# iucario/WorkoutDetector

Measured on AMD Instinct MI355X. Metric: clips/sec (8x3x224x224 TSM-R50), higher is better.
Workload: dtype f32

## Files before the change

### workoutdetector_amd/csrc/tsm_engine.hip

```cpp
#include <hip/hip_runtime.h>

#include <sys/stat.h>

#include <algorithm>
#include <cerrno>
#include <cmath>
#include <cstdio>
#include <cstdlib>
#include <cstring>
#include <map>
#include <string>
#include <vector>

#include "../../include/tsm_hip.h"
#include "tsm_host_util.h"
#include "tsm_kernels.h"

#ifndef TSM_BUILD_ID
#define TSM_BUILD_ID __DATE__ "/" __TIME__
#endif

namespace {

using namespace tsm_host;
// ... 97 lines not shown
  std::string err;
  hipStream_t stream = nullptr;
  bool finalized = false;
  int prec = tsm::kPrecF32;
  float *d_tap = nullptr;
  std::map<std::string, HostTensor> tensors;
  std::vector<ConvLayer> convs;
  std::vector<Block> blocks;
  float *d_fcw = nullptr, *d_fcb = nullptr;
  float *d_in = nullptr;
  float *d_in4 = nullptr;
  float *buf[5] = {nullptr, nullptr, nullptr, nullptr, nullptr};
  float *d_pooled = nullptr, *d_logits = nullptr;
  float *d_partial = nullptr;
  size_t partial_elems = 0;
  size_t buf_elems = 0;
  int h1 = 0, w1 = 0, hp = 0, wp = 0;
  hipEvent_t ev0 = nullptr, ev1 = nullptr;
  bool have_time = false;
  std::vector<void *> allocs;
  bool poison = false;
  std::vector<GuardBuf> guards;
  std::map<int, std::vector<int>> tile_cache;
  bool autotune = true;
  bool stem_pool = true;
  bool stem_direct = true;
  bool stem_planar = true;
  std::string tune_path, tune_sig;
  int force_tile = 0, force_code = -1;
  int fuse23 = -1;
  int fuse_block = -1;
  int fuse31 = -1;
  int fuse_front = -1;
  int walk = -1;
  int n_cu = 256;
  int timing_left = 0;
  bool timing_only3x3 = false;
  std::vector<std::vector<hipEvent_t>> timing;
  std::vector<hipEvent_t> event_pool;
  std::vector<hipEvent_t> *cur_timing = nullptr;
};

namespace {

int fail(tsm_engine *e, int code, const std::string &msg) {
  if (e) e->err = msg; else g_create_error = msg;
  return code;
}

#define TSM_HIP(e, call)                                                                        \
  do {                                                                                          \
    hipError_t _st = (call);                                                                    \
    if (_st != hipSuccess)                                                                      \
      return fail((e), TSM_ERR_HIP, std::string(#call) + ": " + hipGetErrorString(_st));        \
  } while (0)

void build_topology(tsm_engine *e) {
  e->convs.clear();
  e->blocks.clear();
  ConvLayer stem;
  stem.wkey = "base_model.conv1.weight";
  stem.bnp = "base_model.bn1";
  stem.cin = 3; stem.cout = 64; stem.k = 7; stem.stride = 2;
  stem.cp = 4;
  stem.kp = e->prec == tsm::kPrecF32 ? round_up(7 * 7 * 4, 32) : round_up(7 * 4 * 8, e->prec == tsm::kPrecBf16 ? 64 : 32);
  e->convs.push_back(stem);
// ... 342 lines not shown
            tsm::bneck_ws_valid(L.pb.cin, L.pb.N, L.pb.H, L.pb.W, L.pb.T, L.pb.fold) && !want(".conv1") && !want(".conv2");
  f.front = bf16 && blk.stride == 2 && c1.cin == 256 && c1.cout == 128 && c2.cin == 128 && c2.cout == 128 && e->fuse_front != 0 &&
            tsm::front_s2_valid(L.pfr.N, L.pfr.H, L.pfr.W, L.pfr.T, L.pfr.fold) && !want(".conv1");
  f.conv23 = (blk.d_w3f != nullptr || (bf16 && blk.cmid == 64 && tsm::conv23_ws_valid(nn, hh, ww))) && e->fuse23 != 0 &&
             !want(".conv2");
  f.conv31 = bf16 && blk.down < 0 && k + 1 < e->blocks.size() && e->blocks[k + 1].conv3 >= 0 && e->fuse31 != 0 &&
             tsm::conv31_valid(L.q);
  return f;
}

struct BlockPlan {
  bool block = false, front = false, conv1_done = false, conv23 = false, conv31_next = false;
};

std::vector<BlockPlan> plan_forward(const tsm_engine *e, const std::vector<int> *codes, int nn, const char *stage) {
  std::vector<BlockPlan> plan(e->blocks.size());
  int hh = e->hp, ww = e->wp;
  for (size_t k = 0; k < e->blocks.size(); ++k) {
    const Block &blk = e->blocks[k];
    const BlockForms can = fused_forms(e, k, nn, hh, ww, stage);
    auto chosen = [&](int force, int conv, int bit) { return force == 1 || (codes && ((*codes)[conv] & bit)); };
    BlockPlan &p = plan[k];
    p.conv1_done = k > 0 && plan[k - 1].conv31_next;
    if (can.block && chosen(e->fuse_block, blk.conv1, kCodeBlock)) p.block = true;
    else if (can.front && !p.conv1_done && chosen(e->fuse_front, blk.conv1, kCodeFront)) p.front = true;
    else if (can.conv23 && chosen(e->fuse23, blk.conv2, kCodeConv23)) p.conv23 = true;
    else if (can.conv31 && chosen(e->fuse31, blk.conv3, kCodeConv31)) p.conv31_next = true;
    hh = (hh + 2 - 3) / blk.stride + 1;
    ww = (ww + 2 - 3) / blk.stride + 1;
  }
  return plan;
}

struct Forward {
  tsm_engine *e;
  hipStream_t s;
  const char *stage;
  Tap *tap;
  int T, shiftT, prec;
  float *t1, *t2, *idb;
  std::vector<int> *tiles = nullptr;
  bool tuning = false;
  bool tapped = false;
  int flip = 0;
  int prev31 = -1;
  BlockLaunches prev;

  Forward(tsm_engine *e_, hipStream_t s_, const char *stage_, Tap *tap_)
      : e(e_), s(s_), stage(stage_), tap(tap_), T(e_->cfg.num_segments), shiftT(e_->cfg.is_shift ? T : 0), prec(e_->prec),
        t1(e_->buf[2]), t2(e_->buf[3]), idb(e_->buf[4]) {}

  int dir(int d) const { return e->walk >= 0 ? e->walk : d; }
  int next_dir() { return dir(flip ^= 1); }
  bool want(const std::string &name) const { return stage && name == stage; }
  int hit(const float *p, int64_t a, int64_t b, int64_t c, int64_t d) {
    tap->ptr = p; tap->shape[0] = a; tap->shape[1] = b; tap->shape[2] = c; tap->shape[3] = d; tap->hit = true;
    tapped = true;
    return TSM_OK;
  }
  hipError_t launch_code(tsm::ConvParams p, int ks, int code);
  hipError_t launch_pair(const tsm::ConvParams &a, int ks_a, int code_a, const tsm::ConvParams &b, int ks_b, int code_b) {
    const hipError_t st = launch_code(a, ks_a, code_a);
    return st != hipSuccess ? st : launch_code(b, ks_b, code_b);
  }
  template <class A, class B>
  int fused_wins(A &&many, B &&one, bool *wins) {
    float many_ms = 0.f, one_ms = 0.f;
    int rc = time_best_of(e, s, many, &many_ms);
    if (!rc) rc = time_best_of(e, s, one, &one_ms);
    *wins = one_ms < many_ms;
    return rc;
  }
  int conv(int idx, tsm::ConvParams p, int ks, bool is3x3);
  int run_basic(size_t k, int nn, float *x, float *y, int hh, int ww);
  int run_block(size_t k, const BlockPlan &plan, int nn, float *x, float *y, int hh, int ww);
  int tune_block(size_t k, int nn, float *x, float *y, int hh, int ww);
};

hipError_t Forward::launch_code(tsm::ConvParams p, int ks, int code) {
  return launch_conv_code(p, ks, code, e->d_partial, e->partial_elems, e->n_cu, s);
}

int Forward::conv(int idx, tsm::ConvParams p, int ks, bool is3x3) {
  p.reverse = next_dir();
  if (!tuning) {
    int code = tiles ? (*tiles)[idx] : 0;
    if (e->force_tile) code = e->force_tile;
    if (e->force_code >= 0) code = e->force_code;
    TSM_LAUNCH_K(e, s, is3x3, launch_code(p, ks, checked_code(p, code)));
    return TSM_OK;
  }
  std::vector<int> cands;
  if (p.kseg_len > 0) {
    const size_t need = (size_t)tsm::conv_num_segments(p) * p.M * p.Cout;
    const long tiles64 = (long)((p.M + 63) / 64) * (p.Cout / 64);
    for (int t : {(int)tsm::kTile64x64, (int)tsm::kTile32x32}) {
      cands.push_back(t);
      if (need <= e->partial_elems && tiles64 < 4L * e->n_cu) cands.push_back(t | kCodeSplitK);
    }
    int tail_from = 0;
    if (tail_split_from(p, e->n_cu, e->partial_elems, &tail_from)) cands.push_back((int)tsm::kTile64x64 | kCodeTailK);
  } else {
    for (int t = 1; t < tsm::kNumTiles; ++t)
      if (tsm::conv_tile_valid(p, t)) cands.push_back(t);
  }
  float best_ms = 0.f;
  int best = 0;
  for (int t : cands) {
    float ms = 0.f;
    const int rc = time_best_of(e, s, [&] { return launch_code(p, ks, t); }, &ms);
    if (rc) return rc;
    if (best == 0 || ms < best_ms) {
      best = t;
      best_ms = ms;
    }
  }
  (*tiles)[idx] = best;
  return TSM_OK;
}

int Forward::run_basic(size_t k, int nn, float *x, float *y, int hh, int ww) {
  const Block &blk = e->blocks[k];
  const std::string &name = blk.name;
  const ConvLayer &c1 = e->convs[blk.conv1], &c2 = e->convs[blk.conv2];
  const int ho = (hh + 2 - 3) / blk.stride + 1, wo = (ww + 2 - 3) / blk.stride + 1;
  const float *identity = x;
  if (blk.down >= 0) {
    tsm::ConvParams pd = make_params(e->convs[blk.down], x, nullptr, idb, nn, hh, ww, false, block_shift(e) ? shiftT : 0,
                                     e->cfg.shift_div, prec);
    int rcd = conv(blk.down, pd, 1, false);
    if (rcd) return rcd;
    identity = idb;
  }
  tsm::ConvParams p1 = make_params(c1, x, nullptr, t1, nn, hh, ww, true, shiftT, e->cfg.shift_div, prec);
  int rc1 = conv(blk.conv1, p1, 3, true);
  if (rc1) return rc1;
  if (want(name + ".conv1")) return hit(t1, nn, ho, wo, c1.cout);
// ... 6 lines not shown
  if (rc2) return rc2;
  if (want(name)) return hit(y, nn, ho, wo, c2.cout);
  return TSM_OK;
}

int Forward::run_block(size_t k, const BlockPlan &plan, int nn, float *x, float *y, int hh, int ww) {
  const Block &blk = e->blocks[k];
  const std::string &name = blk.name;
  const int c1out = e->convs[blk.conv1].cout, c2out = e->convs[blk.conv2].cout, c3out = e->convs[blk.conv3].cout;
  const int ho = (hh + 2 - 3) / blk.stride + 1, wo = (ww + 2 - 3) / blk.stride + 1;
  BlockLaunches L = block_launches(e, k, nn, x, y, t1, t2, hh, ww);
  if (blk.down >= 0) skip_slots(e, 1);
  if (plan.block) {
    L.pb.reverse = next_dir();
    TSM_LAUNCH(e, s, tsm::launch_bneck_ws(L.pb, s));
    skip_slots(e, 2);
    return want(name) ? hit(y, nn, ho, wo, c3out) : TSM_OK;
  }
  if (plan.front) {
    L.pfr.reverse = next_dir();
    TSM_LAUNCH(e, s, tsm::launch_front_s2(L.pfr, s));
    next_dir();
    skip_slots(e, 1);
  } else {
    if (plan.conv1_done) {
      skip_slots(e, 1);
    } else {
      int rc1 = conv(blk.conv1, L.p1, 1, false);
      if (rc1) return rc1;
    }
    if (want(name + ".conv1")) return hit(t1, nn, hh, ww, c1out);
    if (plan.conv23) {
      L.pf.reverse = next_dir();
      TSM_LAUNCH_K(e, s, true, tsm::launch_conv23_fused(L.pf, blk.cmid, blk.cout3, prec, s));
      skip_slots(e, 1);
      return want(name) ? hit(y, nn, ho, wo, c3out) : TSM_OK;
    }
    int rc2 = conv(blk.conv2, L.p2, 3, true);
    if (rc2) return rc2;
  }
  if (want(name + ".conv2")) return hit(t2, nn, ho, wo, c2out);
  if (plan.conv31_next) {
    L.q.reverse = next_dir();
    TSM_LAUNCH(e, s, tsm::launch_conv31_fused(L.q, s));
  } else {
    int rc3 = conv(blk.conv3, L.p3, 1, false);
    if (rc3) return rc3;
  }
  return want(name) ? hit(y, nn, ho, wo, c3out) : TSM_OK;
}

int Forward::tune_block(size_t k, int nn, float *x, float *y, int hh, int ww) {
  const Block &blk = e->blocks[k];
  std::vector<int> &codes = *tiles;
  const BlockForms can = fused_forms(e, k, nn, hh, ww, nullptr);
  BlockLaunches L = block_launches(e, k, nn, x, y, t1, t2, hh, ww);
  const int r1 = flip ^ 1;
  bool wins = false;
  int rc = conv(blk.conv1, L.p1, 1, false);
  if (rc) return rc;
  L.p1.reverse = dir(r1);
  if (prev31 >= 0 && e->fuse31 < 0) {
    const int conv3 = e->blocks[prev31].conv3, code3 = codes[conv3], code1 = codes[blk.conv1];
    tsm::ConvParams pc = L.p1;
    pc.reverse = dir(prev.p3.reverse ^ 1);
    prev.q.reverse = prev.p3.reverse;
    rc = fused_wins([&] { return launch_pair(prev.p3, 1, code3, pc, 1, code1); },
                    [&] { return tsm::launch_conv31_fused(prev.q, s); }, &wins);
    if (rc) return rc;
    if (wins) codes[conv3] |= kCodeConv31;
  }
  rc = conv(blk.conv2, L.p2, 3, true);
  if (rc) return rc;
  L.p2.reverse = dir(r1 ^ 1);
  if (can.front && e->fuse_front < 0) {
    const int code1 = codes[blk.conv1], code2 = codes[blk.conv2];
    L.pfr.reverse = dir(r1);
    rc = fused_wins([&] { return launch_pair(L.p1, 1, code1, L.p2, 3, code2); },
                    [&] { return tsm::launch_front_s2(L.pfr, s); }, &wins);
    if (rc) return rc;
    if (wins) codes[blk.conv1] |= kCodeFront;
  }
  rc = conv(blk.conv3, L.p3, 1, false);
  if (rc) return rc;
  L.p3.reverse = dir(r1);
  prev31 = can.conv31 ? (int)k : -1;
  prev = L;
  const int code1 = codes[blk.conv1], code2 = codes[blk.conv2], code3 = codes[blk.conv3];
  L.pf.reverse = dir(r1 ^ 1);
  L.pb.reverse = dir(r1);
  auto pair = [&] { return launch_pair(L.p2, 3, code2, L.p3, 1, code3); };
  auto fused23 = [&] { return tsm::launch_conv23_fused(L.pf, blk.cmid, blk.cout3, prec, s); };
  bool use_fused = can.conv23 && e->fuse23 == 1;
  if (can.conv23 && e->fuse23 < 0) {
    rc = fused_wins(pair, fused23, &use_fused);
    if (rc) return rc;
    if (use_fused) codes[blk.conv2] |= kCodeConv23;
  }
  if (can.block && e->fuse_block < 0) {
    rc = fused_wins([&] {
      const hipError_t st = launch_code(L.p1, 1, code1);
      return st != hipSuccess ? st : use_fused ? fused23() : pair();
    }, [&] { return tsm::launch_bneck_ws(L.pb, s); }, &wins);
    if (rc) return rc;
    if (wins) codes[blk.conv1] |= kCodeBlock;
  }
  return TSM_OK;
}

int run_forward(tsm_engine *e, const float *d_clips, int layout, int n_clips, float *d_logits,
                hipStream_t s, const char *stage, Tap *tap) {
  const tsm_config &cfg = e->cfg;
  const int T = cfg.num_segments, n = n_clips * T;
  Forward f(e, s, stage, tap);
  if (e->autotune && !stage) {
    auto it = e->tile_cache.find(tile_bucket(n_clips) * T);
    if (it == e->tile_cache.end()) {
      it = e->tile_cache.emplace(tile_bucket(n_clips) * T, std::vector<int>(e->convs.size(), 0)).first;
      f.tuning = true;
    }
    f.tiles = &it->second;
  }

  const int prec = e->prec;
  const float *in4 = e->d_in4;
  const bool pool_stem = e->stem_direct && e->stem_pool && !f.want("conv1");
  const bool planar = layout == TSM_LAYOUT_NTCHW && e->stem_planar && pool_stem && !f.want("input") &&
                      (double)cfg.height * cfg.width * 12.0 < 2.0e9 && (reinterpret_cast<uintptr_t>(d_clips) & 15u) == 0;
  if (layout >= TSM_LAYOUT_NTHWC4 || planar) {
    in4 = d_clips;
// ... 131 lines not shown
  if (cfg->height < 32 || cfg->width < 32)
    return fail(nullptr, TSM_ERR_INVALID_ARG, "height/width must be >= 32");
  {
    const int64_t rows = (int64_t)cfg->max_clips * cfg->num_segments * ((cfg->height + 1) / 2) * ((cfg->width + 1) / 2);
    if (rows >= (int64_t)1 << 31)
      return fail(nullptr, TSM_ERR_CAPACITY, "max_clips * num_segments * (H/2) * (W/2) must stay below 2^31");
  }
  if (cfg->shift_div <= 0 || (64 % cfg->shift_div) != 0 || (64 / cfg->shift_div) % 4 != 0)
    return fail(nullptr, TSM_ERR_UNSUPPORTED, "shift_div must divide 64 with fold % 4 == 0 (8 or 16... )");
  if (cfg->dtype != TSM_DTYPE_F32 && cfg->dtype != TSM_DTYPE_BF16X3 && cfg->dtype != TSM_DTYPE_BF16)
    return fail(nullptr, TSM_ERR_UNSUPPORTED, "dtype must be TSM_DTYPE_F32, TSM_DTYPE_BF16X3 or TSM_DTYPE_BF16");
  if (cfg->dtype != TSM_DTYPE_F32 && (64 / cfg->shift_div) % 8 != 0)
    return fail(nullptr, TSM_ERR_UNSUPPORTED, "the bf16 formats need fold % 8 == 0 (shift_div <= 8)");
  int ndev = 0;
  hipError_t st = hipGetDeviceCount(&ndev);
  if (st != hipSuccess || ndev <= 0)
    return fail(nullptr, TSM_ERR_HIP, std::string("no HIP device: ") + hipGetErrorString(st));
  if (cfg->device_id < 0 || cfg->device_id >= ndev) return fail(nullptr, TSM_ERR_INVALID_ARG, "bad device_id");
  tsm_engine *e = new tsm_engine();
  e->cfg = *cfg;
  e->prec = cfg->dtype == TSM_DTYPE_BF16X3 ? tsm::kPrecBf16x3
            : cfg->dtype == TSM_DTYPE_BF16 ? tsm::kPrecBf16 : tsm::kPrecF32;
  if (const char *at = getenv("TSM_AUTOTUNE")) e->autotune = atoi(at) != 0;
  if (const char *sd = getenv("TSM_STEM_DIRECT")) e->stem_direct = atoi(sd) != 0;
  if (const char *sp = getenv("TSM_STEM_POOL")) e->stem_pool = atoi(sp) != 0;
  if (const char *pl = getenv("TSM_STEM_PLANAR")) e->stem_planar = atoi(pl) != 0;
  if (const char *ft = getenv("TSM_CONV_TILE")) e->force_tile = tsm::conv_tile_from_name(ft);
  if (const char *fc = getenv("TSM_CONV_CODE")) e->force_code = atoi(fc);
  if (const char *f23 = getenv("TSM_FUSE_CONV23")) e->fuse23 = atoi(f23) != 0;
  if (const char *fb = getenv("TSM_FUSE_BLOCK")) e->fuse_block = atoi(fb) != 0;
  if (const char *f31 = getenv("TSM_FUSE_C3C1")) e->fuse31 = atoi(f31) != 0;
  if (const char *ff = getenv("TSM_FUSE_FRONT")) e->fuse_front = atoi(ff) != 0;
  if (const char *wk = getenv("TSM_WALK")) e->walk = atoi(wk) != 0;
  if (const char *po = getenv("TSM_POISON")) e->poison = atoi(po) != 0;
  {
    const char *tc = getenv("TSM_TUNE_CACHE");
    if (tc) {
      if (*tc && strcmp(tc, "0") != 0 && strcmp(tc, "off") != 0) e->tune_path = tc;
    } else {
      e->tune_path = default_tune_cache_path();
    }
  }
  build_topology(e);
  st = hipSetDevice(cfg->device_id);
  if (st == hipSuccess) st = hipStreamCreateWithFlags(&e->stream, hipStreamNonBlocking);
  if (st == hipSuccess) st = hipDeviceGetAttribute(&e->n_cu, hipDeviceAttributeMultiprocessorCount, cfg->device_id);
  if (st == hipSuccess) st = hipEventCreate(&e->ev0);
  if (st == hipSuccess) st = hipEventCreate(&e->ev1);
  if (st != hipSuccess) {
    g_create_error = std::string("engine init: ") + hipGetErrorString(st);
    delete e;
    return TSM_ERR_HIP;
  }
  if (!e->tune_path.empty()) {
    hipDeviceProp_t prop;
    e->tune_sig = "abi" + std::to_string(TSM_ABI_VERSION) + " build " TSM_BUILD_ID " " +
                  (hipGetDeviceProperties(&prop, cfg->device_id) == hipSuccess ? std::string(prop.gcnArchName) : "?") +
                  " cu" + std::to_string(e->n_cu) +
                  " T" + std::to_string(cfg->num_segments) + " " + std::to_string(cfg->height) + "x" +
                  std::to_string(cfg->width) + " dtype" + std::to_string(cfg->dtype) + " shift" +
                  std::to_string(cfg->is_shift ? cfg->shift_div : 0) + " fuse" + std::to_string(e->fuse23) + "/" + std::to_string(e->fuse_block) + "/" + std::to_string(e->fuse31) + "/" + std::to_string(e->fuse_front) +
                  " stem" + std::to_string(e->stem_direct ? 1 : 0) +
                  std::to_string(e->stem_pool ? 1 : 0) + std::to_string(e->stem_planar ? 1 : 0);
    e->tune_sig_base = e->tune_sig.size();
  }
  *out = e;
  return TSM_OK;
}

int tsm_set_backbone(tsm_engine *e, int32_t depth) {
  if (!e) return TSM_ERR_INVALID_ARG;
  if (e->weights_started || e->finalized)
    return fail(e, TSM_ERR_INVALID_ARG, "tsm_set_backbone must come before the first tsm_set_tensor");
  if (!find_backbone(depth)) return fail(e, TSM_ERR_UNSUPPORTED, "depth must be 18, 34 or 50");
  if (find_backbone(depth)->basic && e->width != 64)
    return fail(e, TSM_ERR_UNSUPPORTED, "a BasicBlock backbone (depth 18 / 34) has no bottleneck width: the engine's is " +
                                            std::to_string(e->width));
  e->depth = depth;
  build_topology(e);
  retag_tune_sig(e);
  return TSM_OK;
}

int tsm_set_bottleneck_width(tsm_engine *e, int32_t width_per_group) {
  if (!e) return TSM_ERR_INVALID_ARG;
  if (e->weights_started || e->finalized)
    return fail(e, TSM_ERR_INVALID_ARG, "tsm_set_bottleneck_width must come before the first tsm_set_tensor");
  if (width_per_group != 64 && width_per_group != 128)
    return fail(e, TSM_ERR_UNSUPPORTED, "width_per_group must be 64 or 128 (wide_resnet50_2)");
  if (width_per_group != 64 && find_backbone(e->depth)->basic)
    return fail(e, TSM_ERR_UNSUPPORTED, "width_per_group 128 needs a Bottleneck backbone (depth 50): torchvision's BasicBlock "
                                        "supports 64 only");
  e->width = width_per_group;
  build_topology(e);
  retag_tune_sig(e);
  return TSM_OK;
// ... 292 lines not shown
  e->timing_only3x3 = only_conv3x3 != 0;
  for (auto &v : e->timing)
    for (hipEvent_t ev : v)
      if (ev) e->event_pool.push_back(ev);
  e->timing.clear();
  e->timing.reserve(64);
  e->timing_left = n_forwards;
  return TSM_OK;
}

int tsm_layer_times(tsm_engine *e, int32_t forward_index, float *ms_out, int32_t cap, int32_t *n_out) {
  if (!e || !ms_out || !n_out) return TSM_ERR_INVALID_ARG;
  if (forward_index < 0 || forward_index >= (int32_t)e->timing.size())
    return fail(e, TSM_ERR_INVALID_ARG, "no timing recorded for that forward");
  const std::vector<hipEvent_t> &ev = e->timing[forward_index];
  const int n = (int)ev.size() / 2;
  *n_out = n;
  if (n > cap) return fail(e, TSM_ERR_CAPACITY, "ms_out too small");
  for (int i = 0; i < n; ++i) {
    ms_out[i] = -1.f;
    if (!ev[2 * i] || !ev[2 * i + 1]) continue;
    TSM_HIP(e, hipEventSynchronize(ev[2 * i + 1]));
    TSM_HIP(e, hipEventElapsedTime(&ms_out[i], ev[2 * i], ev[2 * i + 1]));
  }
  return TSM_OK;
}

int tsm_conv_tiles(tsm_engine *e, int32_t n_clips, int32_t *tiles_out, int32_t cap, int32_t *n_out) {
  if (!e || !tiles_out || !n_out) return TSM_ERR_INVALID_ARG;
  std::vector<int> codes(e->convs.size(), 0);
  auto it = e->tile_cache.find(tile_bucket(n_clips) * e->cfg.num_segments);
  if (it != e->tile_cache.end()) {
    const std::vector<BlockPlan> plan = plan_forward(e, &it->second, n_clips * e->cfg.num_segments, nullptr);
    for (size_t i = 0; i < codes.size(); ++i) codes[i] = it->second[i] & ~kCodeFused;
    for (size_t k = 0; k < e->blocks.size(); ++k) {
      const Block &b = e->blocks[k];
      const BlockPlan &p = plan[k];
      codes[b.conv1] |= it->second[b.conv1] & ((p.block ? kCodeBlock : 0) | (p.front ? kCodeFront : 0));
      if (p.conv23) codes[b.conv2] |= it->second[b.conv2] & kCodeConv23;
      if (p.conv31_next) codes[b.conv3] |= it->second[b.conv3] & kCodeConv31;
    }
  }
  std::vector<int> order{0};
  for (const Block &b : e->blocks)
    for (int ci : {b.down, b.conv1, b.conv2, b.conv3})
      if (ci >= 0) order.push_back(ci);
  *n_out = (int32_t)order.size();
  if ((int)order.size() > cap) return fail(e, TSM_ERR_CAPACITY, "tiles_out too small");
  for (size_t i = 0; i < order.size(); ++i) tiles_out[i] = codes[order[i]];
  return TSM_OK;
}

float tsm_last_forward_ms(tsm_engine *e) {
  if (!e || !e->have_time) return -1.f;
  if (hipEventSynchronize(e->ev1) != hipSuccess) return -1.f;
  float ms = -1.f;
  if (hipEventElapsedTime(&ms, e->ev0, e->ev1) != hipSuccess) return -1.f;
  return ms;
}


int tsm_temporal_shift(const float *x, float *y, int64_t n_frames, int32_t n_segment, int64_t hw, int32_t c,
                       int32_t fold_div, void *stream) {
  if (!x || !y || n_frames <= 0 || hw <= 0 || c <= 0 || fold_div <= 0) return TSM_ERR_INVALID_ARG;
  const int fold = c / fold_div;
  hipError_t st = tsm::launch_temporal_shift(x, y, n_frames, n_segment, hw, c, fold, static_cast<hipStream_t>(stream));
  if (st != hipSuccess) return fail(nullptr, st == hipErrorInvalidValue ? TSM_ERR_INVALID_ARG : TSM_ERR_HIP,
                                    std::string("temporal_shift: ") + hipGetErrorString(st));
  return TSM_OK;
}
// ... 314 lines not shown
```

### workoutdetector_amd/csrc/tsm_fused23.hip

```cpp
#include "tsm_device.h"

namespace tsm {

#define TSM_F23_KERNEL conv23_fused_kernel
#define TSM_F23_NCHUNK 4
#include "tsm_fused23_kernel.h"
#undef TSM_F23_KERNEL
#undef TSM_F23_NCHUNK

#define TSM_F23_KERNEL conv23_fused2_kernel
#define TSM_F23_NCHUNK 2
#include "tsm_fused23_kernel.h"
#undef TSM_F23_KERNEL
#undef TSM_F23_NCHUNK

hipError_t launch_conv23_fused(const Fused23Params &p_in, int cmid, int cout3, int prec, hipStream_t s) {
  Fused23Params p = p_in;
  if (prec == kPrecBf16) {
    if (cmid != 64 || cout3 != 256 || !p.x || !p.w2 || !p.bias2 || !p.w3f || !p.bias3 || !p.res || !p.y || p.M != p.N * p.H * p.W)
      return hipErrorInvalidValue;
    return launch_conv23_ws(p, s);
  }
  if (prec != kPrecF32 && prec != kPrecBf16x3) return hipErrorInvalidValue;
  if (prec == kPrecBf16x3 && p.kseg_len != 0) return hipErrorInvalidValue;
  if (!p.x || !p.w2 || !p.bias2 || !p.w3f || !p.bias3 || !p.res || !p.y) return hipErrorInvalidValue;
  if ((cmid != 64 && cmid != 128) || p.N <= 0 || p.H <= 0 || p.W <= 0 || p.M != p.N * p.H * p.W) return hipErrorInvalidValue;
  if (cout3 != 4 * cmid && !(cout3 == 2 * cmid && cmid == 128)) return hipErrorInvalidValue;
  if (p.kseg_len < 0 || 6.0 * p.H * p.W * cmid * 4.0 > 2.0e9) return hipErrorInvalidValue;
  const unsigned grid = (unsigned)((p.M + 63) / 64);
  if (cout3 == 2 * cmid) {
    if (prec == kPrecBf16x3) TSM_KLAUNCH_WALK(p.reverse, (conv23_fused2_kernel<128, true>), dim3(grid), dim3(512), 0, s, p);
    else TSM_KLAUNCH_WALK(p.reverse, (conv23_fused2_kernel<128, false>), dim3(grid), dim3(512), 0, s, p);
    return hipGetLastError();
  }
  if (prec == kPrecBf16x3) {
    if (cmid == 64) TSM_KLAUNCH_WALK(p.reverse, (conv23_fused_kernel<64, true>), dim3(grid), dim3(256), 0, s, p);
    else TSM_KLAUNCH_WALK(p.reverse, (conv23_fused_kernel<128, true>), dim3(grid), dim3(512), 0, s, p);
  } else {
    if (cmid == 64) TSM_KLAUNCH_WALK(p.reverse, (conv23_fused_kernel<64, false>), dim3(grid), dim3(256), 0, s, p);
    else TSM_KLAUNCH_WALK(p.reverse, (conv23_fused_kernel<128, false>), dim3(grid), dim3(512), 0, s, p);
  }
  return hipGetLastError();
}

}
```

### workoutdetector_amd/csrc/tsm_host_util.h

```cpp
#pragma once
#include <cmath>
#include <cstddef>
#include <cstdint>
#include <cstdio>
#include <cstdlib>
#include <cstring>
#include <string>
#include <vector>

namespace tsm_host {

constexpr float kBnEps = 1e-5f;

inline int segment_len(int kp, int prec) {
  if (prec != 0 ) return 0;
  const int nk = kp / 32;
  if (nk < 32) return 0;
  const int nseg = nk / 16;
  return (nk + nseg - 1) / nseg;
}

inline int round_up(int v, int m) { return (v + m - 1) / m * m; }

inline long tail_split_point(long m_rows, int cout, int n_seg, int n_cu, size_t scratch_elems, int wg_per_cu = 5) {
  if (m_rows <= 0 || cout <= 0 || cout % 64 != 0 || n_seg < 2 || n_cu <= 0) return 0;
  const long ntn = cout / 64, ntm = (m_rows + 63) / 64, tiles = ntm * ntn, slots = (long)wg_per_cu * n_cu;
  const long rounds = tiles / slots, rem = tiles - rounds * slots;
  if (rounds < 1 || rem == 0 || rem * 100 > slots * 85) return 0;
  const long from = rounds * slots / ntn * ntn;
  if (from <= 0 || from >= tiles) return 0;
  const size_t tail_rows = (size_t)(m_rows - (from / ntn) * 64);
  if ((size_t)n_seg * tail_rows * (size_t)cout > scratch_elems) return 0;
  return from;
}

inline uint16_t f2bf(float f) {
  uint32_t u;
  std::memcpy(&u, &f, 4);
  if ((u & 0x7fffffffu) > 0x7f800000u) return (uint16_t)((u >> 16) | 0x40);
  u += 0x7fffu + ((u >> 16) & 1u);
  return (uint16_t)(u >> 16);
}
inline float bf2f(uint16_t h) {
  const uint32_t u = (uint32_t)h << 16;
  float f;
  std::memcpy(&f, &u, 4);
  return f;
}
inline void to_bf16(std::vector<float> *v) {
  std::vector<float> out((v->size() + 1) / 2, 0.f);
  uint16_t *o = reinterpret_cast<uint16_t *>(out.data());
  for (size_t i = 0; i < v->size(); ++i) o[i] = f2bf((*v)[i]);
  v->swap(out);
}
inline void to_split(std::vector<float> *v) {
  uint16_t g[16];
  for (size_t i = 0; i + 8 <= v->size(); i += 8) {
    for (int e = 0; e < 8; ++e) {
      const float x = (*v)[i + e];
      g[e] = f2bf(x);
      g[8 + e] = f2bf(x - bf2f(g[e]));
    }
    std::memcpy(v->data() + i, g, 32);
  }
}

// ... 98 lines not shown
        for (int lane = 0; lane < 64; ++lane)
          for (int s = 0; s < 4; ++s) {
            const int n = j * cmid + wn * 32 + (lane & 31), k = 8 * kk + 4 * (lane >> 5) + s;
            (*out)[((((size_t)j * wgn + wn) * nkk + kk) * 64 + lane) * 4 + s] = w3p[(size_t)n * cmid + k];
          }
}

inline void pack_w3_fragments_split(const float *w3p, int cmid, std::vector<float> *out, int nchunk = 4) {
  const int wgn = cmid / 32, nkq = cmid / 16;
  out->assign((size_t)nchunk * cmid * cmid, 0.f);
  uint16_t *o = reinterpret_cast<uint16_t *>(out->data());
  for (int j = 0; j < nchunk; ++j)
    for (int wn = 0; wn < wgn; ++wn)
      for (int kq = 0; kq < nkq; ++kq)
        for (int lane = 0; lane < 64; ++lane) {
          const int n = j * cmid + wn * 32 + (lane & 31), k0 = 16 * kq + 8 * (lane >> 5);
          const size_t base = ((((size_t)j * wgn + wn) * (2 * nkq) + 2 * kq) * 64 + lane) * 8;
          for (int e = 0; e < 8; ++e) {
            const float x = w3p[(size_t)n * cmid + k0 + e];
            const uint16_t hi = f2bf(x);
            o[base + e] = hi;
            o[base + 64 * 8 + e] = f2bf(x - bf2f(hi));
          }
        }
}

constexpr int kCodeTileMask = 0xF;
constexpr int kCodeSplitK = 0x100;
constexpr int kCodeTailK = 0x200;
constexpr int kCodeConv23 = 0x400;
constexpr int kCodeBlock = 0x800;
constexpr int kCodeConv31 = 0x1000;
constexpr int kCodeFront = 0x2000;
constexpr int kCodeFused = kCodeConv23 | kCodeBlock | kCodeConv31 | kCodeFront;
constexpr int kCodeValid = kCodeTileMask | kCodeSplitK | kCodeTailK | kCodeFused;

inline bool parse_tune_line(const char *line, const std::string &want, int num_tiles, std::vector<int> *codes) {
  if (strncmp(line, want.c_str(), want.size()) != 0) return false;
  std::vector<int> got;
  const char *q = line + want.size();
  while (*q && *q != '\n') {
    char *end = nullptr;
    const long v = strtol(q, &end, 10);
    if (end == q) return false;
    if (v < 0 || (v & ~(long)kCodeValid) != 0 || (int)(v & kCodeTileMask) >= num_tiles) return false;
    got.push_back((int)v);
    if (*end == ',') q = end + 1;
    else if (*end == '\n' || *end == 0) q = end;
    else return false;
  }
  if (got.size() != codes->size()) return false;
  *codes = got;
  return true;
}

}
```

### workoutdetector_amd/csrc/tsm_igemm.hip

```cpp
#include "tsm_device.h"

namespace tsm {

template <int BM, int BN, int WGM, int WGN, int KS, bool SHIFT, bool RES, int PREC, bool DUAL = false, bool SEG = false>
__global__ void __launch_bounds__(64 * WGM * WGN, (SEG && BM == 64) ? ((PREC & kPrecBlockShift) ? 4 : 5) : 1)
conv_igemm(const ConvParams p) {
  constexpr bool BSHIFT = (PREC & kPrecBlockShift) != 0;
  constexpr int PMODE = PREC & ~kPrecBlockShift;
  static_assert(!BSHIFT || (!SHIFT && !RES), "block placement: a shifted identity (DUAL = false) or a shifted second source");
  constexpr bool RESID = RES || (BSHIFT && !DUAL);
  static_assert(!SEG || (PMODE == kPrecF32 && !RES && WGM * WGN <= 4 && BM == BN && BM <= 64),
                "segmented K accumulation: fp32, 64x64 / 32x32 tiles, no residual (ConvParams::kseg_len)");
  static_assert(WGM * WGN == 4 || WGM * WGN == 1 || WGM * WGN == 8,
                "4 waves per workgroup, 1 (32x32 small-M tiles) or 8 (128x128 with 4 waves per SIMD at 2 workgroups/CU)");
  constexpr int NT = 64 * WGM * WGN;
  constexpr int LRP = NT / 8;
  static_assert(!DUAL || (KS == 1 && !SHIFT && !RES), "K-concatenated second source: plain 1x1 convs only");
  constexpr bool X3 = PMODE == kPrecBf16x3;
  constexpr bool BF = PMODE == kPrecBf16;
  constexpr int EB = BF ? 2 : 4;
  constexpr int KC = 128 / EB;
  static_assert(!SHIFT || KS == 1 || (KS == 3 && !SEG), "the temporal shift is fused into 1x1 and unsegmented 3x3 convs only");
  constexpr int WTM = BM / WGM, WTN = BN / WGN;
  constexpr int TM = WTM / 32, TN = WTN / 32;
// ... 772 lines not shown
hipError_t launch_conv(const ConvParams &p_in, int ks, hipStream_t s) {
  ConvParams p = p_in;
  const int kc = p.prec == kPrecBf16 ? 64 : kBK;
  if (p.Cout % 64 != 0 || p.Kp % kc != 0 || p.M <= 0) return hipErrorInvalidValue;
  if ((1 << p.logC4) * 4 != p.C) return hipErrorInvalidValue;
  if (ks != 7 && p.C % kc != 0) return hipErrorInvalidValue;
  if (p.T > 0 && ((ks != 1 && ks != 3) || (ks == 3 && p.kseg_len > 0) || p.N % p.T != 0 || p.fold % 4 != 0 ||
                  (p.res && 2 * p.fold > p.Cout) || (p.x2 && 2 * p.fold > p.C2)))
    return hipErrorInvalidValue;
  if (p.x2 && (ks != 1 || p.res || p.K1 % kc != 0 || p.C2 % kc != 0 || p.K1 + p.C2 != p.Kp || p.K1 != p.C))
    return hipErrorInvalidValue;
  if (p.x2 && (128.0 / ((double)p.Ho * p.Wo) + 4.0) * (double)p.Hi2 * p.Wi2 * p.C2 * 4.0 > 2.0e9) return hipErrorInvalidValue;
  if (p.T > 0 && p.res && (128.0 + 2.0 * p.Ho * p.Wo) * p.Cout * 4.0 > 2.0e9) return hipErrorInvalidValue;
  if (p.prec != kPrecF32 && p.prec != kPrecBf16x3 && p.prec != kPrecBf16) return hipErrorInvalidValue;
  if (p.kseg_len < 0 || (p.kseg_len > 0 && (p.prec != kPrecF32 || p.res || ks == 7))) return hipErrorInvalidValue;
  if ((p.ksplit && p.kseg_len <= 0) || p.ksplit < 0 || p.ksplit > 2) return hipErrorInvalidValue;
  if (p.prec != kPrecF32 && p.T > 0 && p.fold % 8 != 0) return hipErrorInvalidValue;
  if (ks == 7 && (p.C != 4 || (p.prec != kPrecF32 && (p.stride != 2 || p.pad != 3)))) return hipErrorInvalidValue;
  const double frames = 128.0 / ((double)p.Ho * p.Wo) + 4.0;
  if (frames * (double)p.Hi * p.Wi * p.C * 4.0 > 2.0e9) return hipErrorInvalidValue;
  switch (ks) {
    case 1:
      if (p.res) return launch_conv_ks<1, false, true>(p, s);
      return p.T > 0 && !p.x2 ? launch_conv_ks<1, true, false>(p, s) : launch_conv_ks<1, false, false>(p, s);
    case 3:
      if (p.res) return launch_conv_ks<3, false, true>(p, s);
      return p.T > 0 ? launch_conv_ks<3, true, false>(p, s) : launch_conv_ks<3, false, false>(p, s);
    case 7: return p.res ? hipErrorInvalidValue : launch_conv_ks<7, false, false>(p, s);
    default: return hipErrorInvalidValue;
  }
}


__global__ void __launch_bounds__(256) splitk_reduce_kernel(const float *__restrict__ partial, int n_seg, int64_t n4,
                                                            int64_t seg_stride4, int cout4,
                                                            const float *__restrict__ bias, const float *__restrict__ res,
                                                            float *__restrict__ y, int relu) {
  const int64_t stride = (int64_t)gridDim.x * blockDim.x;
  const float floor_ = relu ? 0.f : -INFINITY;
  const f32x4 *p4 = reinterpret_cast<const f32x4 *>(partial);
  for (int64_t i = (int64_t)blockIdx.x * blockDim.x + threadIdx.x; i < n4; i += stride) {
    f32x4 t = p4[i];
    for (int sgm = 1; sgm < n_seg; ++sgm) t += p4[i + sgm * seg_stride4];
    f32x4 v = t + reinterpret_cast<const f32x4 *>(bias)[i % cout4];
    if (res) v += reinterpret_cast<const f32x4 *>(res)[i];
    v[0] = fmaxf(v[0], floor_);
    v[1] = fmaxf(v[1], floor_);
    v[2] = fmaxf(v[2], floor_);
    v[3] = fmaxf(v[3], floor_);
    reinterpret_cast<f32x4 *>(y)[i] = v;
  }
}


hipError_t launch_splitk_reduce(const float *partial, int n_seg, int64_t m, int cout, const float *bias,
                                const float *res, float *y, int relu, hipStream_t s) {
  if (!partial || !bias || !y || n_seg < 1 || m <= 0 || cout <= 0 || cout % 4 != 0) return hipErrorInvalidValue;
  const int64_t n4 = m * cout / 4;
  TSM_KLAUNCH(splitk_reduce_kernel, dim3(grid_for(n4, 2048)), dim3(256), 0, s, partial, n_seg, n4, n4, cout / 4,
                     bias, res, y, relu);
  return hipGetLastError();
}

}
```

### workoutdetector_amd/csrc/tsm_kernels.h

```cpp
#pragma once
#include <hip/hip_runtime.h>
#include <stdint.h>

namespace tsm {

struct ConvParams {
  const float *x;
  const float *w;
  const float *bias;
  const float *res;
  float *y;
  int N, Hi, Wi, C, logC4;
  int Ho, Wo, Cout;
  int stride, pad;
  int Kp;
  int M;
  int relu;
  int T;
  int fold;
  int ntm, ntn;
  int tile;
  int prec;
  const float *x2;
  int C2, Hi2, Wi2, stride2;
// ... 9 lines not shown
constexpr int kPrecBlockShift = 4;

enum ConvTile {
  kTileAuto = 0, kTile128x128 = 1, kTile128x64 = 2, kTile64x64 = 3, kTile32x32 = 4,
  kTile128x128w8 = 5,
  kTile256x256 = 6,
  kTileWs = 7,
  kTile256x256p = 8,
  kNumTiles = 9
};
void conv_tile_dims(int tile, int *bm, int *bn);
int conv_tile_from_name(const char *name);
bool conv_tile_valid(const ConvParams &p, int tile);
bool conv3x3_ws_valid(const ConvParams &p);
bool conv3x3_ws128_valid(const ConvParams &p);
bool conv1x1_wsn_valid(const ConvParams &p);
bool conv1x1_ws_valid(const ConvParams &p);

hipError_t launch_conv(const ConvParams &p, int ks, hipStream_t s);
struct Fused23Params {
  const float *x;
  const float *w2;
  const float *bias2;
  const float *w3f;
  const float *bias3;
  const float *res;
  float *y;
  int N, H, W;
  int M;
  int kseg_len;
  int reverse;
};
hipError_t launch_conv23_fused(const Fused23Params &p, int cmid, int cout3, int prec, hipStream_t s);
bool conv23_ws_valid(int n, int h, int w);

struct BneckParams {
  const void *x;
  const void *w1;
  const float *bias1;
  const void *w2;
  const float *bias2;
  const void *w3;
  const float *bias3;
  void *y;
  int cin;
  int N, H, W;
  int T, fold;
  int reverse;
};
bool bneck_ws_valid(int cin, int n, int h, int w, int T, int fold);
hipError_t launch_bneck_ws(const BneckParams &p, hipStream_t s);

struct FrontParams {
  const void *x;
  const void *w1;
  const float *bias1;
  const void *w2;
  const float *bias2;
  void *y;
  int N, H, W;
  int T, fold;
  int reverse;
};
bool front_s2_valid(int n, int h, int w, int T, int fold);
hipError_t launch_front_s2(const FrontParams &p, hipStream_t s);

// ... 84 lines not shown
```

### workoutdetector_amd/engine.py

```python
from __future__ import annotations

import ctypes as C
from dataclasses import dataclass
from typing import Dict, List, Mapping, Optional, Sequence

import numpy as np

from . import _lib
from .weights import (BACKBONES, DEPTHS, SHIFT_PLACES, WIDTHS, is_mmaction_state_dict, make_state_dict, remap_checkpoint_keys,
                      remap_mmaction_keys)

CONSENSUS_TYPES = {'avg': 0, 'identity': 1}


@dataclass
class NodeArg:
    name: str
    shape: list
    type: str = 'tensor(float)'


def _as_f32(a) -> np.ndarray:
    return np.ascontiguousarray(np.asarray(a), dtype=np.float32)

# ... 166 lines not shown
    def forward_tap(self, clips: np.ndarray, stage: str) -> np.ndarray:
        self._need_finalized()
        clips = _as_f32(clips)
        self._check_clips(clips.size, clips.shape[0], _lib.LAYOUT_NTCHW)
        n = clips.shape[0] * self.num_segments
        h1, w1 = (self.height - 1) // 2 + 1, (self.width - 1) // 2 + 1
        hp, wp = (h1 - 1) // 2 + 1, (w1 - 1) // 2 + 1
        cap = n * max(h1 * w1 * 64, hp * wp * 256, self.height * self.width * 8)
        buf = np.empty(cap, dtype=np.float32)
        shape = (C.c_int64 * 4)()
        _lib.check(self._lib.tsm_forward_tap(self._h, clips.ctypes.data, _lib.MEM_HOST, _lib.LAYOUT_NTCHW,
                                             clips.shape[0], stage.encode(), buf.ctypes.data, cap, shape, None),
                   self._h)
        dims = tuple(int(v) for v in shape)
        return buf[:int(np.prod(dims))].reshape(dims).copy()

    def launch_names(self) -> List[str]:
        names = ['pack_input', 'conv1', 'maxpool']
        blocks, kind = BACKBONES[self.base_model]
        for li, nb in enumerate(blocks, start=1):
            for b in range(nb):
                p = f'layer{li}.{b}'
                if kind == 'basic':
                    names += ([p + '.downsample'] if b == 0 and li > 1 else []) + [p + '.conv1', p + '.conv2']
                else:
                    names += ([p + '.downsample'] if b == 0 else []) + [p + '.conv1', p + '.conv2', p + '.conv3']
        return names + ['head']

    TILE_NAMES = {0: 'heuristic', 1: '128x128', 2: '128x64', 3: '64x64', 4: '32x32', 5: '128x128w8', 6: '256x256', 7: 'ws',
                  8: '256x256p'}

    @classmethod
    def tile_name(cls, code: int) -> str:
        return (cls.TILE_NAMES[code & 15] + ('/splitK' if code & 0x100 else '') + ('/tailK' if code & 0x200 else '') + ('+conv3' if code & 0x400 else '') +
                ('+block' if code & 0x800 else '') + ('+conv1' if code & 0x1000 else '') + ('+conv2' if code & 0x2000 else ''))

    def conv_tiles(self, n_clips: int) -> Dict[str, str]:
        buf = (C.c_int32 * 64)()
        n = C.c_int32()
        _lib.check(self._lib.tsm_conv_tiles(self._h, n_clips, buf, 64, C.byref(n)), self._h)
        names = [k for k in self.launch_names() if k not in ('pack_input', 'maxpool', 'head')]
        assert n.value == len(names)
        return {k: self.tile_name(buf[i]) for i, k in enumerate(names)}

    def set_layer_timing(self, n_forwards: int, only_conv3x3: bool = False) -> None:
        _lib.check(self._lib.tsm_set_layer_timing(self._h, n_forwards, int(only_conv3x3)), self._h)

    def layer_times_ms(self, forward_index: int) -> Dict[str, float]:
        buf = (C.c_float * 80)()
        n = C.c_int32()
        _lib.check(self._lib.tsm_layer_times(self._h, forward_index, C.addressof(buf), 80, C.byref(n)), self._h)
        names = self.launch_names()
        assert n.value == len(names), (n.value, len(names))
        return {k: float(buf[i]) for i, k in enumerate(names)}

    @property
    def last_forward_ms(self) -> float:
        return float(self._lib.tsm_last_forward_ms(self._h))

    def _need_finalized(self) -> None:
        if not self._finalized:
            raise _lib.TsmError(-3, 'load_state_dict() has not been called')

    def close(self) -> None:
        if getattr(self, '_h', None) is not None and self._h.value:
            self._lib.tsm_destroy(self._h)
            self._h = C.c_void_p()
# ... 280 lines not shown
```

Before: 1843.

## Split partial-wave frame tails onto smaller tiles for 1x1 and fused conv23

Adds a frame-tail split: when a 128x128 1x1 conv or fused conv2+conv3 launch would leave a partially filled last wave, the frames are cut at a wave boundary computed from occupancy queries. Full waves run the original kernel and the remaining frames run with 64x64 tiles (split-K for the 3x3). The split is added as an autotuning candidate flagged with a new code bit. It aims to reduce wave-quantization idle time, at the cost of an extra launch and more tuning work.

```diff
diff --git a/workoutdetector_amd/csrc/tsm_engine.hip b/workoutdetector_amd/csrc/tsm_engine.hip
--- a/workoutdetector_amd/csrc/tsm_engine.hip
+++ b/workoutdetector_amd/csrc/tsm_engine.hip
@@ -153,6 +153,10 @@
   int fuse_block = -1;
   int fuse31 = -1;
   int fuse_front = -1;
+  int frame_tail = -1;
+  long tail_slots = 0;
+  int wg_f23[2] = {0, 0};
+  int wg_128[2][3] = {{0, 0, 0}, {0, 0, 0}};
   int walk = -1;
   int n_cu = 256;
   int timing_left = 0;
@@ -561,6 +565,53 @@
   return plan;
 }
 
+long chip_slots(const tsm_engine *e, int wg_per_cu) { return e->tail_slots > 0 ? e->tail_slots : (long)wg_per_cu * e->n_cu; }
+
+int frame_tail_conv(const tsm_engine *e, const tsm::ConvParams &p, int ks, int code) {
+  if (e->frame_tail == 0 || e->prec != tsm::kPrecF32 || ks != 1 || p.kseg_len > 0 || p.x2 || p.stride != 1 || p.Cout % 128 != 0 ||
+      (p.T > 0 && p.res))
+    return 0;
+  if (e->frame_tail < 0 && !(code & kCodeTailF)) return 0;
+  int tile = code & kCodeTileMask;
+  if (tile == tsm::kTileAuto) {
+    int bm = 0, bn = 0;
+    tsm::conv_tile_shape(p, &bm, &bn);
+    if (bm != 128 || bn != 128) return 0;
+    tile = tsm::kTile128x128;
+  }
+  if (tile != tsm::kTile128x128 && tile != tsm::kTile128x128w8) return 0;
+  const int wg = e->wg_128[tile == tsm::kTile128x128w8 ? 1 : 0][p.res ? 2 : p.T > 0 ? 1 : 0];
+  return (int)tsm_host::frame_tail_point(p.N, (long)p.Ho * p.Wo, p.T > 0 ? p.T : 1, 128, p.Cout / 128, chip_slots(e, wg));
+}
+
+int frame_tail_conv23(const tsm_engine *e, const Block &blk, const tsm::Fused23Params &pf, int code2) {
+  if (e->frame_tail == 0 || e->prec != tsm::kPrecF32 || !blk.d_w3f || blk.cout3 != 4 * blk.cmid) return 0;
+  if (e->frame_tail < 0 && !(code2 & kCodeTailF)) return 0;
+  return (int)tsm_host::frame_tail_point(pf.N, (long)pf.H * pf.W, 1, 64, 1, chip_slots(e, e->wg_f23[blk.cmid == 128 ? 1 : 0]));
+}
+
+int conv23_tail_code(const tsm_engine *e, int code2) {
+  if (e->force_tile) code2 &= ~kCodeTailF;
+  if (e->force_code >= 0) code2 = (code2 & ~kCodeTailF) | (e->force_code & kCodeTailF);
+  return code2;
+}
+
+void note_frame_tail(int frames, int f0, bool tail_first) {
+  char text[96];
+  snprintf(text, sizeof text, " [frames = %d, f0 = %d, %s]", frames, f0, tail_first ? "tail first" : "head first");
+  tsm::note_launch("frame_tail", text);
+}
+
+tsm::ConvParams conv_frames(tsm::ConvParams p, int f0, int f1) {
+  const size_t in_off = (size_t)f0 * p.Hi * p.Wi * p.C, out_off = (size_t)f0 * p.Ho * p.Wo * p.Cout;
+  p.x += in_off;
+  if (p.res) p.res += out_off;
+  p.y += out_off;
+  p.N = f1 - f0;
+  p.M = p.N * p.Ho * p.Wo;
+  return p;
+}
+
 struct Forward {
   tsm_engine *e;
   hipStream_t s;
@@ -588,6 +639,7 @@
     return TSM_OK;
   }
   hipError_t launch_code(tsm::ConvParams p, int ks, int code);
+  hipError_t launch_conv23(const BlockLaunches &L, const Block &blk, int f0);
   hipError_t launch_pair(const tsm::ConvParams &a, int ks_a, int code_a, const tsm::ConvParams &b, int ks_b, int code_b) {
     const hipError_t st = launch_code(a, ks_a, code_a);
     return st != hipSuccess ? st : launch_code(b, ks_b, code_b);
@@ -607,7 +659,38 @@
 };
 
 hipError_t Forward::launch_code(tsm::ConvParams p, int ks, int code) {
-  return launch_conv_code(p, ks, code, e->d_partial, e->partial_elems, e->n_cu, s);
+  const int f0 = frame_tail_conv(e, p, ks, code);
+  code &= ~kCodeTailF;
+  if (f0 <= 0) return launch_conv_code(p, ks, code, e->d_partial, e->partial_elems, e->n_cu, s);
+  const int head_code = (code & kCodeTileMask) == tsm::kTileAuto ? (int)tsm::kTile128x128 : (code & kCodeTileMask);
+  const tsm::ConvParams head = conv_frames(p, 0, f0), tail = conv_frames(p, f0, p.N);
+  note_frame_tail(p.N, f0, p.reverse != 0);
+  hipError_t st = hipSuccess;
+  for (int part = 0; part < 2 && st == hipSuccess; ++part)
+    st = (part == 0) == (p.reverse != 0) ? launch_conv_code(tail, ks, tsm::kTile64x64, e->d_partial, e->partial_elems, e->n_cu, s)
+                                         : launch_conv_code(head, ks, head_code, e->d_partial, e->partial_elems, e->n_cu, s);
+  return st;
+}
+
+hipError_t Forward::launch_conv23(const BlockLaunches &L, const Block &blk, int f0) {
+  if (f0 <= 0) return tsm::launch_conv23_fused(L.pf, blk.cmid, blk.cout3, prec, s);
+  tsm::Fused23Params head = L.pf;
+  head.N = f0;
+  head.M = f0 * head.H * head.W;
+  tsm::ConvParams c2 = conv_frames(L.p2, f0, L.pf.N), c3 = conv_frames(L.p3, f0, L.pf.N);
+  c2.reverse = L.pf.reverse;
+  c3.reverse = dir(L.pf.reverse ^ 1);
+  note_frame_tail(L.pf.N, f0, L.pf.reverse != 0);
+  hipError_t st = hipSuccess;
+  for (int part = 0; part < 2 && st == hipSuccess; ++part) {
+    if ((part == 0) == (L.pf.reverse != 0)) {
+      st = launch_conv_code(c2, 3, (int)tsm::kTile64x64 | kCodeSplitK, e->d_partial, e->partial_elems, e->n_cu, s);
+      if (st == hipSuccess) st = launch_conv_code(c3, 1, tsm::kTile64x64, e->d_partial, e->partial_elems, e->n_cu, s);
+    } else {
+      st = tsm::launch_conv23_fused(head, blk.cmid, blk.cout3, prec, s);
+    }
+  }
+  return st;
 }
 
 int Forward::conv(int idx, tsm::ConvParams p, int ks, bool is3x3) {
@@ -632,6 +715,9 @@
   } else {
     for (int t = 1; t < tsm::kNumTiles; ++t)
       if (tsm::conv_tile_valid(p, t)) cands.push_back(t);
+    for (int t : {(int)tsm::kTile128x128, (int)tsm::kTile128x128w8})
+      if (e->frame_tail < 0 && tsm::conv_tile_valid(p, t) && frame_tail_conv(e, p, ks, t | kCodeTailF) > 0)
+        cands.push_back(t | kCodeTailF);
   }
   float best_ms = 0.f;
   int best = 0;
@@ -704,7 +790,8 @@
     if (want(name + ".conv1")) return hit(t1, nn, hh, ww, c1out);
     if (plan.conv23) {
       L.pf.reverse = next_dir();
-      TSM_LAUNCH_K(e, s, true, tsm::launch_conv23_fused(L.pf, blk.cmid, blk.cout3, prec, s));
+      const int f0 = frame_tail_conv23(e, blk, L.pf, conv23_tail_code(e, tiles ? (*tiles)[blk.conv2] : 0));
+      TSM_LAUNCH_K(e, s, true, launch_conv23(L, blk, f0));
       skip_slots(e, 1);
       return want(name) ? hit(y, nn, ho, wo, c3out) : TSM_OK;
     }
@@ -762,12 +849,23 @@
   L.pf.reverse = dir(r1 ^ 1);
   L.pb.reverse = dir(r1);
   auto pair = [&] { return launch_pair(L.p2, 3, code2, L.p3, 1, code3); };
-  auto fused23 = [&] { return tsm::launch_conv23_fused(L.pf, blk.cmid, blk.cout3, prec, s); };
+  const int forced_f0 = e->frame_tail == 1 ? frame_tail_conv23(e, blk, L.pf, 0) : 0;
+  auto fused23 = [&] { return launch_conv23(L, blk, forced_f0); };
   bool use_fused = can.conv23 && e->fuse23 == 1;
   if (can.conv23 && e->fuse23 < 0) {
     rc = fused_wins(pair, fused23, &use_fused);
     if (rc) return rc;
     if (use_fused) codes[blk.conv2] |= kCodeConv23;
+  }
+  const int f0 = can.conv23 && e->frame_tail < 0 && blk.cmid == 128 ? frame_tail_conv23(e, blk, L.pf, kCodeTailF) : 0;
+  if (f0 > 0) {
+    auto split = [&] { return launch_conv23(L, blk, f0); };
+    rc = use_fused ? fused_wins(fused23, split, &wins) : fused_wins(pair, split, &wins);
+    if (rc) return rc;
+    if (wins) {
+      codes[blk.conv2] |= kCodeConv23 | kCodeTailF;
+      use_fused = true;
+    }
   }
   if (can.block && e->fuse_block < 0) {
     rc = fused_wins([&] {
@@ -965,6 +1063,8 @@
   if (const char *f31 = getenv("TSM_FUSE_C3C1")) e->fuse31 = atoi(f31) != 0;
   if (const char *ff = getenv("TSM_FUSE_FRONT")) e->fuse_front = atoi(ff) != 0;
   if (const char *wk = getenv("TSM_WALK")) e->walk = atoi(wk) != 0;
+  if (const char *ft = getenv("TSM_FRAME_TAIL")) e->frame_tail = atoi(ft) != 0;
+  if (const char *ts = getenv("TSM_TAIL_SLOTS")) e->tail_slots = std::max(0L, std::min(atol(ts), 1L << 24));
   if (const char *po = getenv("TSM_POISON")) e->poison = atoi(po) != 0;
   {
     const char *tc = getenv("TSM_TUNE_CACHE");
@@ -978,6 +1078,11 @@
   st = hipSetDevice(cfg->device_id);
   if (st == hipSuccess) st = hipStreamCreateWithFlags(&e->stream, hipStreamNonBlocking);
   if (st == hipSuccess) st = hipDeviceGetAttribute(&e->n_cu, hipDeviceAttributeMultiprocessorCount, cfg->device_id);
+  if (st == hipSuccess && e->prec == tsm::kPrecF32 && e->frame_tail != 0) {
+    for (int c = 0; c < 2; ++c) e->wg_f23[c] = tsm::conv23_fused_wg_per_cu(c ? 128 : 64);
+    for (int w8 = 0; w8 < 2; ++w8)
+      for (int v = 0; v < 3; ++v) e->wg_128[w8][v] = tsm::conv1x1_128_wg_per_cu(w8 != 0, v == 1, v == 2);
+  }
   if (st == hipSuccess) st = hipEventCreate(&e->ev0);
   if (st == hipSuccess) st = hipEventCreate(&e->ev1);
   if (st != hipSuccess) {
@@ -994,7 +1099,8 @@
                   std::to_string(cfg->width) + " dtype" + std::to_string(cfg->dtype) + " shift" +
                   std::to_string(cfg->is_shift ? cfg->shift_div : 0) + " fuse" + std::to_string(e->fuse23) + "/" + std::to_string(e->fuse_block) + "/" + std::to_string(e->fuse31) + "/" + std::to_string(e->fuse_front) +
                   " stem" + std::to_string(e->stem_direct ? 1 : 0) +
-                  std::to_string(e->stem_pool ? 1 : 0) + std::to_string(e->stem_planar ? 1 : 0);
+                  std::to_string(e->stem_pool ? 1 : 0) + std::to_string(e->stem_planar ? 1 : 0) +
+                  " ftail" + std::to_string(e->frame_tail) + "/" + std::to_string(e->tail_slots);
     e->tune_sig_base = e->tune_sig.size();
   }
   *out = e;
@@ -1353,10 +1459,23 @@
   auto it = e->tile_cache.find(tile_bucket(n_clips) * e->cfg.num_segments);
   if (it != e->tile_cache.end()) {
     const std::vector<BlockPlan> plan = plan_forward(e, &it->second, n_clips * e->cfg.num_segments, nullptr);
-    for (size_t i = 0; i < codes.size(); ++i) codes[i] = it->second[i] & ~kCodeFused;
+    for (size_t i = 0; i < codes.size(); ++i) codes[i] = it->second[i] & ~(kCodeFused | kCodeTailF);
+    int hh = e->hp, ww = e->wp;
     for (size_t k = 0; k < e->blocks.size(); ++k) {
       const Block &b = e->blocks[k];
       const BlockPlan &p = plan[k];
+      if (b.conv3 >= 0) {
+        const BlockLaunches L = block_launches(e, k, n_clips * e->cfg.num_segments, e->buf[0], e->buf[1], e->buf[2], e->buf[3], hh, ww);
+        const std::vector<int> &raw = it->second;
+        if (!p.block && !p.front && !p.conv1_done && (raw[b.conv1] & kCodeTailF) && frame_tail_conv(e, L.p1, 1, raw[b.conv1]) > 0)
+          codes[b.conv1] |= kCodeTailF;
+        if (p.conv23 && (conv23_tail_code(e, raw[b.conv2]) & kCodeTailF) && frame_tail_conv23(e, b, L.pf, raw[b.conv2]) > 0)
+          codes[b.conv2] |= kCodeTailF;
+        if (!p.block && !p.conv23 && !p.conv31_next && (raw[b.conv3] & kCodeTailF) && frame_tail_conv(e, L.p3, 1, raw[b.conv3]) > 0)
+          codes[b.conv3] |= kCodeTailF;
+      }
+      hh = (hh + 2 - 3) / b.stride + 1;
+      ww = (ww + 2 - 3) / b.stride + 1;
       codes[b.conv1] |= it->second[b.conv1] & ((p.block ? kCodeBlock : 0) | (p.front ? kCodeFront : 0));
       if (p.conv23) codes[b.conv2] |= it->second[b.conv2] & kCodeConv23;
       if (p.conv31_next) codes[b.conv3] |= it->second[b.conv3] & kCodeConv31;
diff --git a/workoutdetector_amd/csrc/tsm_fused23.hip b/workoutdetector_amd/csrc/tsm_fused23.hip
--- a/workoutdetector_amd/csrc/tsm_fused23.hip
+++ b/workoutdetector_amd/csrc/tsm_fused23.hip
@@ -43,4 +43,14 @@
   return hipGetLastError();
 }
 
+int conv23_fused_wg_per_cu(int cmid) {
+  int n = 0;
+  hipError_t st = hipErrorInvalidValue;
+  if (cmid == 64)
+    st = hipOccupancyMaxActiveBlocksPerMultiprocessor(&n, reinterpret_cast<const void *>(&conv23_fused_kernel<64, false>), 256, 0);
+  else if (cmid == 128)
+    st = hipOccupancyMaxActiveBlocksPerMultiprocessor(&n, reinterpret_cast<const void *>(&conv23_fused_kernel<128, false>), 512, 0);
+  return st == hipSuccess && n > 0 ? n : 0;
 }
+
+}
diff --git a/workoutdetector_amd/csrc/tsm_host_util.h b/workoutdetector_amd/csrc/tsm_host_util.h
--- a/workoutdetector_amd/csrc/tsm_host_util.h
+++ b/workoutdetector_amd/csrc/tsm_host_util.h
@@ -32,6 +32,20 @@
   const size_t tail_rows = (size_t)(m_rows - (from / ntn) * 64);
   if ((size_t)n_seg * tail_rows * (size_t)cout > scratch_elems) return 0;
   return from;
+}
+
+inline long frame_tail_point(long frames, long rows_per_frame, long frames_per_unit, long tile_rows, long ntn, long slots) {
+  if (frames <= 0 || rows_per_frame <= 0 || frames_per_unit <= 0 || tile_rows <= 0 || ntn <= 0 || slots <= 0) return 0;
+  if (frames > (1L << 22) || rows_per_frame > (1L << 20) || tile_rows > (1L << 16) || ntn > (1L << 12) || slots > (1L << 24))
+    return 0;
+  const int64_t tiles = ((int64_t)frames * rows_per_frame + tile_rows - 1) / tile_rows * ntn;
+  const int64_t rounds = tiles / slots, rem = tiles - rounds * slots;
+  if (rounds < 1 || rem == 0 || rem * 100 > (int64_t)slots * 85) return 0;
+  const int64_t head_rows = rounds * slots / ntn * tile_rows;
+  const int64_t f0 = head_rows / rows_per_frame / frames_per_unit * frames_per_unit;
+  if (f0 <= 0 || f0 >= frames) return 0;
+  if ((f0 * rows_per_frame + tile_rows - 1) / tile_rows * ntn < slots) return 0;
+  return (long)f0;
 }
 
 inline uint16_t f2bf(float f) {
@@ -196,8 +210,9 @@
 constexpr int kCodeBlock = 0x800;
 constexpr int kCodeConv31 = 0x1000;
 constexpr int kCodeFront = 0x2000;
+constexpr int kCodeTailF = 0x80;
 constexpr int kCodeFused = kCodeConv23 | kCodeBlock | kCodeConv31 | kCodeFront;
-constexpr int kCodeValid = kCodeTileMask | kCodeSplitK | kCodeTailK | kCodeFused;
+constexpr int kCodeValid = kCodeTileMask | kCodeSplitK | kCodeTailK | kCodeTailF | kCodeFused;
 
 inline bool parse_tune_line(const char *line, const std::string &want, int num_tiles, std::vector<int> *codes) {
   if (strncmp(line, want.c_str(), want.size()) != 0) return false;
diff --git a/workoutdetector_amd/csrc/tsm_igemm.hip b/workoutdetector_amd/csrc/tsm_igemm.hip
--- a/workoutdetector_amd/csrc/tsm_igemm.hip
+++ b/workoutdetector_amd/csrc/tsm_igemm.hip
@@ -828,6 +828,19 @@
 }
 
 
+template <int WGM, bool SHIFT, bool RES>
+static int occupancy_128() {
+  int n = 0;
+  const hipError_t st = hipOccupancyMaxActiveBlocksPerMultiprocessor(
+      &n, reinterpret_cast<const void *>(&conv_igemm<128, 128, WGM, 2, 1, SHIFT, RES, kPrecF32>), 64 * WGM * 2, 0);
+  return st == hipSuccess && n > 0 ? n : 0;
+}
+int conv1x1_128_wg_per_cu(bool w8, bool shift, bool res) {
+  if (shift && res) return 0;
+  if (w8) return res ? occupancy_128<4, false, true>() : shift ? occupancy_128<4, true, false>() : occupancy_128<4, false, false>();
+  return res ? occupancy_128<2, false, true>() : shift ? occupancy_128<2, true, false>() : occupancy_128<2, false, false>();
+}
+
 __global__ void __launch_bounds__(256) splitk_reduce_kernel(const float *__restrict__ partial, int n_seg, int64_t n4,
                                                             int64_t seg_stride4, int cout4,
                                                             const float *__restrict__ bias, const float *__restrict__ res,
diff --git a/workoutdetector_amd/csrc/tsm_kernels.h b/workoutdetector_amd/csrc/tsm_kernels.h
--- a/workoutdetector_amd/csrc/tsm_kernels.h
+++ b/workoutdetector_amd/csrc/tsm_kernels.h
@@ -65,6 +65,8 @@
   int reverse;
 };
 hipError_t launch_conv23_fused(const Fused23Params &p, int cmid, int cout3, int prec, hipStream_t s);
+int conv23_fused_wg_per_cu(int cmid);
+int conv1x1_128_wg_per_cu(bool w8, bool shift, bool res);
 bool conv23_ws_valid(int n, int h, int w);
 
 struct BneckParams {
diff --git a/workoutdetector_amd/engine.py b/workoutdetector_amd/engine.py
--- a/workoutdetector_amd/engine.py
+++ b/workoutdetector_amd/engine.py
@@ -222,7 +222,8 @@
 
     @classmethod
     def tile_name(cls, code: int) -> str:
-        return (cls.TILE_NAMES[code & 15] + ('/splitK' if code & 0x100 else '') + ('/tailK' if code & 0x200 else '') + ('+conv3' if code & 0x400 else '') +
+        return (cls.TILE_NAMES[code & 15] + ('/splitK' if code & 0x100 else '') + ('/tailK' if code & 0x200 else '') + ('/tailF' if code & 0x80 else '') +
+                ('+conv3' if code & 0x400 else '') +
                 ('+block' if code & 0x800 else '') + ('+conv1' if code & 0x1000 else '') + ('+conv2' if code & 0x2000 else ''))
 
     def conv_tiles(self, n_clips: int) -> Dict[str, str]:
```

After: 1846, median of 6. No clear change (+0.2%).
